# fabriceo/AVDSP

Hardware: NVIDIA B200
Metric: channel-samples/sec (higher is better)
Workload: dtype int64

## Files before the change

avdsp_b200/csrc/api.cu:

```cuda
#include "../../include/avdsp_b200.h"
#include "decoder.h"
#include "kernels.h"
#include "host_numa.h"
#include <cuda_runtime.h>
#include <algorithm>
#include <cstdio>
#include <cstdlib>
#include <cstring>
#include <memory>
#include <map>
#include <mutex>
#include <string>
#include <thread>
#include <vector>

using namespace avdsp;

static thread_local std::string g_lastError;
static int setErr(int code, const std::string& msg) { g_lastError = msg; return code; }
static int cudaErr(cudaError_t e, const char* what) {
    return setErr(AVDSP_B200_ERR_CUDA, std::string(what) + ": " + cudaGetErrorString(e));
}
#define NO_MULTI(h, what) do { if (!(h)->shards.empty()) return setErr(AVDSP_B200_ERR_UNSUPPORTED, what " takes a single-device instance (device buffers belong to one GPU)"); } while (0)
#define CU(call) do { cudaError_t e_ = (call); if (e_ != cudaSuccess) return cudaErr(e_, #call); } while (0)
// ... 77 lines not shown
__global__ void k_widen_pcm(const unsigned char* __restrict__ src, int fmt, int* __restrict__ dst, size_t n) {
    const size_t i = (size_t)blockIdx.x * blockDim.x + threadIdx.x;
    if (i >= n) return;
    int v;
    if (fmt == AVDSP_B200_PCM_S16) v = (int)((const short*)src)[i] << 16;
    else { const unsigned char* p = src + 3 * i; v = (int)(((unsigned)p[0] << 8) | ((unsigned)p[1] << 16) | ((unsigned)p[2] << 24)); }
    dst[i] = v;
}

#include "instance.h"

static int quiesce(avdsp_b200* h);
static int resetShards(avdsp_b200* h, int fs, const int32_t* seeds, int defaultDither);

static void planGeometries(avdsp_b200* h, std::vector<ChainLane>* lanes2) {
    const Lowered& L = h->L;
    h->chain2Usable = false;
    lanes2->assign(1024, ChainLane{});
    if (L.chainOk && chain2Supports(L.chain)) h->chain2Usable = planChain2Geometry(L.chain, h->nStreams, h->numSMs, &h->geom2, lanes2->data());
    h->chain3Usable = h->chain2Usable && planChain3Geometry(L.chain, h->nStreams, h->numSMs, &h->geom3);
    h->mixUsable = false;
    if (L.chainOk) { std::string why; h->mixUsable = buildMixPlan(L.chain, &h->mix, &why); }
    h->firUsable = L.firOk;
    h->dagUsable = L.dagOk && L.dag && planDagGeometry(*L.dag, h->nStreams, h->numSMs, &h->geomDag);
    char line[512];
    h->trace = L.trace;
    if (h->firUsable) {
        snprintf(line, sizeof line, "time-parallel FIR kernel: usable (%d paths, longest impulse %d taps)\n", L.fir.nPaths, L.fir.maxLen);
        h->trace += line;
    } else if (!L.firs.empty()) h->trace += "FIR kernel not used: " + L.firWhyNot + "\n";
    if (h->mixUsable) h->trace += "time-parallel mix kernel: usable (no biquad in any path)\n";
    if (h->chain2Usable) {
        snprintf(line, sizeof line, "chain kernel v2 geometry: %d streams/CTA, %d sections/lane, tile %d frames, gmax %d, %d section threads + %d helper threads, %d sources, %zu B smem\n",
                 h->geom2.streamsPerCta, h->geom2.secPerLane, h->geom2.tileFrames, h->geom2.gmax, h->geom2.secThreads, h->geom2.helpThreads, L.chain.h.nSrc, h->geom2.smemBytes);
        h->trace += line;
    }
    if (h->chain3Usable) {
        snprintf(line, sizeof line, "chain kernel v3 geometry: %d streams/CTA (lane = one cascade part of one stream), %d cascade warps of <= %d sections + 1 dither warp + %d store warps, largest lag %d frames, row ring %d steps, %zu B smem; parts (chain:first+n@base):",
                 h->geom3.streamsPerCta, h->geom3.nCascade, h->geom3.maxSec, h->geom3.nStore, h->geom3.gmax, h->geom3.postRing, h->geom3.smemBytes);
        h->trace += line;
        for (int w = 0; w < h->geom3.nCascade; w++) {
            snprintf(line, sizeof line, " %d:%d+%d@%d", h->geom3.warpChain[w], h->geom3.warpFirstSec[w], h->geom3.warpNsec[w], h->geom3.warpBase[w]);
            h->trace += line;
        }
        h->trace += "; sub-partitions (sections of the cascade warps on hardware warps q, q+4, ..; d = dither warp, s = store warp):";
        for (int q = 0; q < 4; q++) {
            h->trace += q ? " |" : " ";
            for (int id = q; id < h->geom3.threads / 32; id += 4) {
                const int role = h->geom3.warpRole[id];
                if (role >= 0) snprintf(line, sizeof line, " %d", h->geom3.warpNsec[role]);
                else snprintf(line, sizeof line, " %s", role == -1 ? "d" : "s");
                h->trace += line;
            }
        }
        h->trace += "\n";
    }
    if (h->dagUsable) {
        snprintf(line, sizeof line, "DAG kernel geometry: %d nodes (depth %d, longest cascade %d sections), %d streams/CTA, %d threads, tiles of %d frames, input rows of %d frames, %d words/stream, %zu B smem%s\n",
                 L.dag->nNodes, L.dag->maxDepth, L.dag->maxSec, h->geomDag.streamsPerCta, h->geomDag.threads, h->geomDag.tileFrames, h->geomDag.rawMask + 1, h->geomDag.perStreamWords,
                 h->geomDag.smemBytes, (h->chain2Usable || h->mixUsable || h->firUsable) ? " (another fused kernel takes this program first)" : "");
        h->trace += line;
    } else if (!L.dagOk && !h->chain2Usable && !h->mixUsable && !h->firUsable) h->trace += "DAG kernel not used: " + L.dagWhyNot + "\n";
    if (!h->chain2Usable && !h->mixUsable) {
        const bool coefRange = L.chainOk && L.chain.h.aluClass == ALU_F32 && !chainFloatCoefsInRange(L.chain);
        snprintf(line, sizeof line, "chain kernels not used: %s\n",
                 coefRange ? "a biquad coefficient lies outside [2^-60, 2^7): the float class could not bound its products (exactness guard), the interpreter runs this program"
                           : L.chainOk ? "geometry does not fit" : L.chainWhyNot.c_str());
        h->trace += line;
    }
}

static int uploadPlanData(avdsp_b200* h) {
    cudaSetDevice(h->device);
    const Lowered& L = h->L;
    if (h->dBig) { cudaFree(h->dBig); h->dBig = nullptr; }
    h->bigWords = L.bigPool.size();
    if (h->bigWords) {
        CU(cudaMalloc(&h->dBig, h->bigWords * 4));
        CU(cudaMemcpy(h->dBig, L.bigPool.data(), h->bigWords * 4, cudaMemcpyHostToDevice));
    }
    std::vector<ChainLane> lanes2;
    planGeometries(h, &lanes2);
    if (h->chain2Usable) {
        if (!h->dLanes2) CU(cudaMalloc(&h->dLanes2, 1024 * sizeof(ChainLane)));
        CU(cudaMemcpy(h->dLanes2, lanes2.data(), 1024 * sizeof(ChainLane), cudaMemcpyHostToDevice));
    }
    if (h->dFirTaps) { cudaFree(h->dFirTaps); h->dFirTaps = nullptr; }
    if (h->firUsable) {
        std::vector<unsigned char> blobs;
        firTcBuildTaps(L.fir, L.fir.aluClass == ALU_INT64 ? FIRTC_I8 : FIRTC_TF32, L.bigPool.data(), &blobs);
        CU(cudaMalloc(&h->dFirTaps, blobs.size()));
        CU(cudaMemcpy(h->dFirTaps, blobs.data(), blobs.size(), cudaMemcpyHostToDevice));
    }
    return 0;
}

static int initState(avdsp_b200* h) {
    cudaSetDevice(h->device);
    const PlanHeader& P = h->L.gen.h;
    const size_t words = (size_t)h->nStreams * P.stateWords;
    CU(cudaMemsetAsync(h->dState, 0, words * 4, h->stream));
    std::vector<int32_t> memInit(2 * std::max(P.nMem, 1), 0);
    for (int k = 0; k < P.nMem; k++) {
        memInit[2 * k] = h->L.words[h->L.memWord[k]];
        memInit[2 * k + 1] = h->L.words[h->L.memWord[k] + 1];
    }
// ... 999 lines not shown
```

avdsp_b200/csrc/kernel_chain3.cu:

```cuda
#include "avdsp_dev.cuh"
#include "kernels.h"
#include <algorithm>
#include <cstdlib>

namespace avdsp {
namespace {

constexpr int F3 = 32;
constexpr int TP3 = 4 * F3 + 1;
constexpr int kBarFull3 = 1;
constexpr int kBarDone3 = 3;
#ifndef AVDSP_UNR3
#define AVDSP_UNR3 6
#endif
constexpr unsigned kSatBias3  = (1u << (kMantBQ - 1)) - 2u;
constexpr unsigned kSatLimit3 = (1u << kMantBQ) - 3u;

__device__ __forceinline__ void barSync3(int id, int n)   { __syncwarp(); asm volatile("bar.sync %0, %1;" :: "r"(id), "r"(n) : "memory"); }
__device__ __forceinline__ void barArrive3(int id, int n) { __syncwarp(); asm volatile("bar.arrive %0, %1;" :: "r"(id), "r"(n) : "memory"); }
__device__ __forceinline__ unsigned smemAddr3(const void* p) { return (unsigned)__cvta_generic_to_shared(p); }
__device__ __forceinline__ int lds3(unsigned a) { int v; asm volatile("ld.shared.b32 %0, [%1];" : "=r"(v) : "r"(a) : "memory"); return v; }
__device__ __forceinline__ void sts3(unsigned a, int v) { asm volatile("st.shared.b32 [%0], %1;" :: "r"(a), "r"(v) : "memory"); }
__device__ __forceinline__ void mbarInit3(unsigned bar, int count) {
    asm volatile("mbarrier.init.shared::cta.b64 [%0], %1;" :: "r"(bar), "r"(count) : "memory");
}
__device__ __forceinline__ void mbarExpectTx3(unsigned bar, unsigned bytes) {
    asm volatile("mbarrier.arrive.expect_tx.shared::cta.b64 _, [%0], %1;" :: "r"(bar), "r"(bytes) : "memory");
}
__device__ __forceinline__ void tmaLoad3(unsigned dst, const void* src, unsigned bytes, unsigned bar) {
    asm volatile("cp.async.bulk.shared::cluster.global.mbarrier::complete_tx::bytes [%0], [%1], %2, [%3];"
                 :: "r"(dst), "l"(src), "r"(bytes), "r"(bar) : "memory");
}
__device__ __forceinline__ void mbarWait3(unsigned bar, unsigned parity) {
    asm volatile("{\n"
                 ".reg .pred P1;\n"
                 "WAIT3_%=:\n"
                 "mbarrier.try_wait.parity.shared::cta.b64 P1, [%0], %1;\n"
                 "@P1 bra DONE3_%=;\n"
                 "bra WAIT3_%=;\n"
                 "DONE3_%=:\n"
                 "}" :: "r"(bar), "r"(parity) : "memory");
}

template <int NSEC>
struct Casc {
    long long acc[NSEC];
    int y1[NSEC], y2[NSEC], y3[NSEC];
    int X1, X2;
    int rx1[NSEC], rx2[NSEC];
    int b0[NSEC], b1[NSEC], b2[NSEC], a1[NSEC], a2[NSEC];
};

template <int NSEC>
__device__ __forceinline__ long long cascStep(Casc<NSEC>& L, int xin, unsigned& w0, unsigned& w1) {
    long long acc[NSEC];
#pragma unroll
    for (int k = 0; k < NSEC; k++) acc[k] = mac32(L.acc[k], k ? L.y2[k - 1] : L.X1, L.b1[k]);
#pragma unroll
    for (int k = 0; k < NSEC; k++) acc[k] = mac32(acc[k], k ? L.y3[k - 1] : L.X2, L.b2[k]);
#pragma unroll
    for (int k = 0; k < NSEC; k++) acc[k] = mac32(acc[k], L.y1[k], L.a1[k]);
#pragma unroll
    for (int k = 0; k < NSEC; k++) acc[k] = mac32(acc[k], L.y2[k], L.a2[k]);
#pragma unroll
    for (int k = 0; k < NSEC; k++) acc[k] = mac32(acc[k], k ? L.y1[k - 1] : xin, L.b0[k]);
#pragma unroll
    for (int k = 0; k < NSEC; k++) {
        if (k & 1) w1 = max(w1, (unsigned)hi32(acc[k]) + kSatBias3);
        else       w0 = max(w0, (unsigned)hi32(acc[k]) + kSatBias3);
        L.acc[k] = acc[k];
        L.y3[k] = L.y2[k]; L.y2[k] = L.y1[k]; L.y1[k] = q59ToS31(acc[k]);
    }
    L.X2 = L.X1; L.X1 = xin;
    return acc[NSEC - 1];
}
template <int NSEC>
__device__ __forceinline__ long long cascStepExact(Casc<NSEC>& L, int xin, int t, int T) {
    int in[NSEC], x1[NSEC], x2[NSEC];
#pragma unroll
    for (int k = 0; k < NSEC; k++) {
        const int f = t - k;
        in[k] = k ? L.y1[k - 1] : xin;
        x1[k] = k ? (f == 0 ? L.rx1[k] : L.y2[k - 1]) : L.X1;
        x2[k] = k ? (f == 0 ? L.rx2[k] : (f == 1 ? L.rx1[k] : L.y3[k - 1])) : L.X2;
    }
    long long last = 0;
#pragma unroll
    for (int k = 0; k < NSEC; k++) {
        if ((unsigned)(t - k) < (unsigned)T) {
            long long acc = L.acc[k];
            acc = mac32(acc, x1[k], L.b1[k]);
            acc = mac32(acc, x2[k], L.b2[k]);
            acc = mac32(acc, L.y1[k], L.a1[k]);
            acc = mac32(acc, L.y2[k], L.a2[k]);
            acc = mac32(acc, in[k], L.b0[k]);
            acc = biquadSat(acc);
            L.acc[k] = acc;
            L.y3[k] = L.y2[k]; L.y2[k] = L.y1[k]; L.y1[k] = q59ToS31(acc);
            if (k == NSEC - 1) last = acc;
        }
    }
    if ((unsigned)t < (unsigned)T) { L.X2 = L.X1; L.X1 = xin; }
    return last;
}

__device__ __forceinline__ int finishTpdf3(long long acc, int tv, bool up, int sh) {
    const long long t = tv;
    acc += up ? (long long)((unsigned long long)t << sh) : (t >> sh);
    return sat64_031_s32(acc);
}

template <int NSEC, int MODE, bool CKREG>
__device__ __forceinline__ void cascadeWarp(const ChainPlan& P, const Chain2Args& A, const Chain3Geom& G, unsigned char* smem,
                                            int w, int lane) {
    constexpr int LAG = NSEC - 1;
    const int NS = G.streamsPerCta, W = P.h.stateWords, T = A.nFrames;
    const int s0 = blockIdx.x * NS, nsHere = min(NS, A.nStreams - s0);
    const int c = G.warpChain[w];
    const ChainDesc& d = P.chains[c];
    const int sec0 = G.warpFirstSec[w];
    const int base = G.warpBase[w];
    const int LAGA = base + LAG;
    const int srcWarp = G.warpSrc[w];
    const bool fin = G.warpFinal[w] != 0;
    const bool live = lane < nsHere;
    const int sl = min(lane, nsHere - 1);
    const int RM = G.postRing - 1;
    const unsigned RM4 = (unsigned)RM << 2, TM4 = (unsigned)(4 * F3 - 1) << 2;
    const unsigned sb = smemAddr3(smem);
    const unsigned postRow = sb + (unsigned)G.warpRowOff[w] + (unsigned)(sl * G.warpPitch[w]) * 4u;
    const unsigned srcRow = sb + (unsigned)G.warpRowOff[max(srcWarp, 0)] + (unsigned)(sl * G.warpPitch[max(srcWarp, 0)]) * 4u;
    volatile int* tileDone = reinterpret_cast<volatile int*>(smem + G.doneOff);
    const unsigned tpdfRow = sb + G.tpdfOff + (unsigned)(sl * TP3) * 4u;
    const unsigned rawRow = sb + G.rawOff + (unsigned)(sl * G.rawPitchBytes) + (unsigned)d.srcCh * 4u;
    const unsigned fb = (unsigned)P.h.nIn * 4u;
    const unsigned mbar = sb + G.mbarOff;
    const int gain = srcWarp >= 0 ? (1 << kMant) : (d.srcKind == SRC_LOAD_GAIN ? d.srcArg : 1);
    const bool tpdfUp = P.h.tpdfShift >= 0;
    const int tpdfSh = (tpdfUp ? P.h.tpdfShift : -P.h.tpdfShift) & 63;
    const bool wantTpdf = fin && (d.satKind & 1) != 0;
    int* st = A.state + (size_t)(s0 + sl) * W;

    Casc<NSEC> L;
    L.X1 = L.X2 = 0;
#pragma unroll
    for (int k = 0; k < NSEC; k++) {
        const int* cf = P.pool + d.coefOff + 5 * (sec0 + k);
        L.b0[k] = cf[0]; L.b1[k] = cf[1]; L.b2[k] = cf[2]; L.a1[k] = cf[3]; L.a2[k] = cf[4];
        L.y3[k] = 0;
        {
            const int* q = st + P.pool[d.secStateOff + sec0 + k];
            L.acc[k] = (long long)(((unsigned long long)(unsigned)q[1] << 32) | (unsigned)q[0]);
            L.rx1[k] = q[2]; L.rx2[k] = q[3]; L.y1[k] = q[4]; L.y2[k] = q[5];
            if (k == 0) { L.X1 = q[2]; L.X2 = q[3]; }
        }
    }
    const int n = fin ? d.delayN : 0;
    int idx0 = 0, staleIdx = -1;
    if (live && n > 0) {
        const int* ring = st + d.delayOff + 1;
        idx0 = st[d.delayOff];
        const bool stale = idx0 >= n || idx0 < 0;
        for (int k = 0; k < n; k++) {
            const int v = !stale ? ring[(idx0 + k) % n] : (k == 0 ? ring[idx0] : ring[k - 1]);
            sts3(postRow + ((unsigned)((k - n + LAGA) & RM) << 2), v);
        }
        if (stale) { sts3(postRow + ((unsigned)(LAGA & RM) << 2), ring[n - 1]); staleIdx = idx0; idx0 = n - 1; }
    }
    const bool anyStale = __any_sync(0xffffffffu, staleIdx >= 0);
    int* ck = reinterpret_cast<int*>(smem + G.ckOff) + (w * 32 + lane);
    const int CKP = G.nCascade * 32;
    const int nTiles = (T + G.gmax + F3 - 1) / F3;

    for (int i = 0; i < nTiles; i++) {
        barSync3(kBarFull3 + (i & 1), G.threads);
        const int t0 = i * F3;
        unsigned ra, rstep;
        if (srcWarp < 0) {
            if (G.tma && t0 + F3 <= T) mbarWait3(mbar + 8u * (unsigned)(i & 1), (unsigned)((i >> 1) & 1));
            ra = rawRow + (unsigned)(i & 1) * (unsigned)G.rawStageBytes; rstep = fb;
        } else {
            if (i > 0) { while (tileDone[srcWarp] < i) { } __threadfence_block(); __syncwarp(); }
            ra = srcRow + (unsigned)(((i + 2) % 3) * F3) * 4u; rstep = 4u;
        }
        const int tl0 = t0 - base;
        bool exact = !(tl0 >= LAG + 2 && tl0 + F3 <= T && !(anyStale && tl0 <= LAG));
        if (!exact) {
            long long cAcc[CKREG ? NSEC : 1]; int cY1[CKREG ? NSEC : 1], cY2[CKREG ? NSEC : 1], cY3[CKREG ? NSEC : 1], cX1 = 0, cX2 = 0;
            if (CKREG) {
#pragma unroll
                for (int k = 0; k < NSEC; k++) { cAcc[CKREG ? k : 0] = L.acc[k]; cY1[CKREG ? k : 0] = L.y1[k]; cY2[CKREG ? k : 0] = L.y2[k]; cY3[CKREG ? k : 0] = L.y3[k]; }
                cX1 = L.X1; cX2 = L.X2;
            } else {
#pragma unroll
                for (int k = 0; k < NSEC; k++) {
                    ck[(5 * k + 0) * CKP] = lo32(L.acc[k]); ck[(5 * k + 1) * CKP] = hi32(L.acc[k]);
                    ck[(5 * k + 2) * CKP] = L.y1[k]; ck[(5 * k + 3) * CKP] = L.y2[k]; ck[(5 * k + 4) * CKP] = L.y3[k];
                }
                ck[(5 * NSEC) * CKP] = L.X1; ck[(5 * NSEC + 1) * CKP] = L.X2;
            }
            unsigned w0 = 0, w1 = 0;
            unsigned rj = ra;
            unsigned pj = postRow + (fin ? ((unsigned)(t0 & RM) << 2) : (unsigned)((i % 3) * F3) * 4u);
            unsigned tj = (unsigned)((t0 - LAGA) << 2);
            auto step = [&](int jj) {
                const int smp = lds3(rj); rj += rstep;
                const int x = (MODE & 1) ? smp : q59ToS31(mul32(smp, gain));
                const long long acc = cascStep<NSEC>(L, x, w0, w1);
                int v;
                if (MODE & 2) v = finishTpdf3(acc, lds3(tpdfRow + ((tj + 4u * jj) & TM4)), tpdfUp, tpdfSh);
                else v = q59ToS31(acc);
                if (live) sts3(pj + 4u * jj, v);
            };
            constexpr int kMain = (F3 / AVDSP_UNR3) * AVDSP_UNR3;
#pragma unroll 1
            for (int j0 = 0; j0 < kMain; j0 += AVDSP_UNR3) {
#pragma unroll
                for (int jj = 0; jj < AVDSP_UNR3; jj++) step(jj);
                pj += 4u * AVDSP_UNR3; tj += 4u * AVDSP_UNR3;
            }
#pragma unroll
            for (int jj = 0; jj < F3 - kMain; jj++) step(jj);
            if (__any_sync(0xffffffffu, max(w0, w1) > kSatLimit3)) {
                if (CKREG) {
#pragma unroll
                    for (int k = 0; k < NSEC; k++) { L.acc[k] = cAcc[CKREG ? k : 0]; L.y1[k] = cY1[CKREG ? k : 0]; L.y2[k] = cY2[CKREG ? k : 0]; L.y3[k] = cY3[CKREG ? k : 0]; }
                    L.X1 = cX1; L.X2 = cX2;
                } else {
#pragma unroll
                    for (int k = 0; k < NSEC; k++) {
                        L.acc[k] = (long long)(((unsigned long long)(unsigned)ck[(5 * k + 1) * CKP] << 32) | (unsigned)ck[(5 * k + 0) * CKP]);
                        L.y1[k] = ck[(5 * k + 2) * CKP]; L.y2[k] = ck[(5 * k + 3) * CKP]; L.y3[k] = ck[(5 * k + 4) * CKP];
                    }
                    L.X1 = ck[(5 * NSEC) * CKP]; L.X2 = ck[(5 * NSEC + 1) * CKP];
                }
                exact = true;
            }
        }
        if (exact) {
#pragma unroll 1
            for (int j = 0; j < F3; j++) {
                const int t = t0 + j, tl = t - base;
                if (tl >= T + LAG) break;
                if (tl < 0) continue;
                const int smp = tl < T ? lds3(ra + (unsigned)j * rstep) : 0;
                const int x = q59ToS31(mul32(smp, gain));
                const long long acc = cascStepExact<NSEC>(L, x, tl, T);
                const int f = tl - LAG;
                if (f >= 0) {
                    int v;
                    if (wantTpdf) v = finishTpdf3(acc, lds3(tpdfRow + ((unsigned)(f << 2) & TM4)), tpdfUp, tpdfSh);
                    else v = q59ToS31(acc);
                    if (live) {
                        if (f == 0 && staleIdx >= 0) st[d.delayOff + 1 + staleIdx] = v;
                        else sts3(postRow + (fin ? ((unsigned)(t << 2) & RM4) : (unsigned)((i % 3) * F3 + j) * 4u), v);
                    }
                }
            }
        }
        if (!fin) {
            __syncwarp();
            if (lane == 0) { __threadfence_block(); tileDone[w] = i + 1; }
        }
        barArrive3(kBarDone3 + (i & 1), G.threads);
    }

    if (live) {
#pragma unroll
        for (int k = 0; k < NSEC; k++) {
            int* q = st + P.pool[d.secStateOff + sec0 + k];
            q[0] = lo32(L.acc[k]); q[1] = hi32(L.acc[k]);
            if (k == 0) { q[2] = L.X1; q[3] = L.X2; }
            else if (T >= 2) { q[2] = L.y1[k - 1]; q[3] = L.y2[k - 1]; }
            else if (T == 1) { q[2] = L.y1[k - 1]; q[3] = L.rx1[k]; }
            q[4] = L.y1[k]; q[5] = L.y2[k];
        }
// ... 253 lines not shown
                if (f >= 0) {
                    const int v = emit(acc, f);
                    if (live) {
                        if (f == 0 && staleIdx >= 0) st[d.delayOff + 1 + staleIdx] = v;
                        else sts3(postRow + (fin ? ((unsigned)(t << 2) & RM4) : (unsigned)((i % 3) * F3 + j) * 4u), v);
                    }
                }
            }
        }
        if (!fin) {
            __syncwarp();
            if (lane == 0) { __threadfence_block(); tileDone[w] = i + 1; }
        }
        barArrive3(kBarDone3 + (i & 1), G.threads);
    }
    if (live) {
#pragma unroll
        for (int k = 0; k < NSEC; k++) {
            int* q = st + P.pool[d.secStateOff + sec0 + k];
            q[0] = __float_as_int(L.acc[k]);
            if (k == 0) { q[2] = __float_as_int(L.X1); q[3] = __float_as_int(L.X2); }
            else if (T >= 2) { q[2] = __float_as_int(L.y1[k - 1]); q[3] = __float_as_int(L.y2[k - 1]); }
            else if (T == 1) { q[2] = __float_as_int(L.y1[k - 1]); q[3] = __float_as_int(L.rx1[k]); }
            q[4] = __float_as_int(L.y1[k]); q[5] = __float_as_int(L.y2[k]);
        }
        if (fltGuardFired(mn) && A.redo) A.redo[s0 + sl] = 1;
        if (n > 0 && T > 0) {
            int* ring = st + d.delayOff + 1;
            for (int k = 0; k < n; k++) {
                const long long j = (long long)T - n + k;
                ring[(int)(((long long)idx0 + j + n) % n)] = __float_as_int(satF(__int_as_float(lds3(postRow + ((unsigned)(((int)j + LAGA) & RM) << 2)))));
            }
            st[d.delayOff] = (int)(((long long)idx0 + T) % n);
        }
    }
}
template <int NSEC>
__device__ __forceinline__ void cascadeWarpFin(const ChainPlan& P, const Chain2Args& A, const Chain3Geom& G, unsigned char* smem, int w, int lane) {
    const int finm = !G.warpFinal[w] ? 0 : (P.chains[G.warpChain[w]].satKind & 1) ? 2 : 1;
    const int src = G.warpSrc[w] >= 0 ? 1 : (P.h.sampleInt ? 0 : 2);
    switch (finm * 3 + src) {
    case 0:  cascadeWarpF<NSEC, 0, 0>(P, A, G, smem, w, lane); break;
    case 1:  cascadeWarpF<NSEC, 0, 1>(P, A, G, smem, w, lane); break;
    case 2:  cascadeWarpF<NSEC, 0, 2>(P, A, G, smem, w, lane); break;
    case 3:  cascadeWarpF<NSEC, 1, 0>(P, A, G, smem, w, lane); break;
    case 4:  cascadeWarpF<NSEC, 1, 1>(P, A, G, smem, w, lane); break;
    case 5:  cascadeWarpF<NSEC, 1, 2>(P, A, G, smem, w, lane); break;
    case 6:  cascadeWarpF<NSEC, 2, 0>(P, A, G, smem, w, lane); break;
    case 7:  cascadeWarpF<NSEC, 2, 1>(P, A, G, smem, w, lane); break;
    default: cascadeWarpF<NSEC, 2, 2>(P, A, G, smem, w, lane); break;
    }
}

template <int NSEC, bool CKREG>
__device__ __forceinline__ void cascadeWarpMode(const ChainPlan& P, const Chain2Args& A, const Chain3Geom& G, unsigned char* smem,
                                                int w, int lane, int mode) {
    switch (mode) {
    case 0:  cascadeWarp<NSEC, 0, CKREG>(P, A, G, smem, w, lane); break;
    case 1:  cascadeWarp<NSEC, 1, CKREG>(P, A, G, smem, w, lane); break;
    case 2:  cascadeWarp<NSEC, 2, CKREG>(P, A, G, smem, w, lane); break;
    default: cascadeWarp<NSEC, 3, CKREG>(P, A, G, smem, w, lane); break;
    }
}

template <bool FLT, bool FSMP> __device__ __forceinline__ int post3(int v) {
    if (FLT) return FSMP ? __float_as_int(satF(__int_as_float(v))) : f2s31SatFast(v);
    return v;
}

template <int NOUT, bool FLT, bool FSMP>
__device__ __forceinline__ void storeTile3(int* __restrict__ out, unsigned rowA, unsigned p4, unsigned RM4, int mask, bool clean,
                                           int f0, int fs, int T) {
    constexpr int FPP = 32 / NOUT, NPASS = F3 / FPP;
    if (clean) {
#pragma unroll
        for (int p = 0; p < NPASS; p++) out[p * 32] = post3<FLT, FSMP>(lds3(rowA + ((p4 + (unsigned)(p * FPP * 4)) & RM4))) & mask;
    } else {
#pragma unroll 1
        for (int p = 0; p < NPASS; p++) {
            const int f = f0 + p * FPP + fs;
            if (f >= 0 && f < T) out[p * 32] = post3<FLT, FSMP>(lds3(rowA + ((p4 + (unsigned)(p * FPP * 4)) & RM4))) & mask;
        }
    }
}

template <int NOUT, bool FLT, bool FSMP>
__device__ __forceinline__ void storeStreams3(int* __restrict__ out, size_t outStep, unsigned rowA, unsigned rowStep, int cnt, unsigned p4,
                                              unsigned RM4, int mask, bool clean, int f0, int fs, int T) {
#pragma unroll 1
    for (int s = 0; s < cnt; s++, out += outStep, rowA += rowStep) storeTile3<NOUT, FLT, FSMP>(out, rowA, p4, RM4, mask, clean, f0, fs, T);
}

}

template <int MAXSEC, bool FLT = false>
__global__ void __launch_bounds__(MAXSEC > 4 ? kChain3MaxThreads : kChain3MaxThreadsParts, 1)
k_chain3(const __grid_constant__ ChainPlan P, const Chain2Args A, const __grid_constant__ Chain3Geom G) {
    extern __shared__ __align__(128) unsigned char smem_raw[];
    const int lane = threadIdx.x & 31;
    const int role = G.warpRole[threadIdx.x >> 5];
    if constexpr (FLT) {
        if (role >= 0) {
            switch (G.warpNsec[role]) {
            case 1: cascadeWarpFin<1>(P, A, G, smem_raw, role, lane); break;
            case 2: cascadeWarpFin<2>(P, A, G, smem_raw, role, lane); break;
            case 3: cascadeWarpFin<3>(P, A, G, smem_raw, role, lane); break;
            default: cascadeWarpFin<4>(P, A, G, smem_raw, role, lane); break;
            }
            return;
        }
    } else if (role >= 0) {
        const int warp = role;
        const ChainDesc& d = P.chains[G.warpChain[warp]];
        const bool unity = G.warpSrc[warp] >= 0 || (d.srcKind == SRC_LOAD_GAIN && d.srcArg == (1 << kMant));
        const int mode = (unity ? 1 : 0) | ((G.warpFinal[warp] && (d.satKind & 1)) ? 2 : 0);
        switch (G.warpNsec[warp]) {
        case 1: cascadeWarpMode<1, (MAXSEC <= 4)>(P, A, G, smem_raw, warp, lane, mode); break;
        case 2: cascadeWarpMode<2, (MAXSEC <= 4)>(P, A, G, smem_raw, warp, lane, mode); break;
        case 3: cascadeWarpMode<3, (MAXSEC <= 4)>(P, A, G, smem_raw, warp, lane, mode); break;
        case 4: cascadeWarpMode<4, (MAXSEC <= 4)>(P, A, G, smem_raw, warp, lane, mode); break;
        default:
            if constexpr (MAXSEC > 4) {
                switch (G.warpNsec[warp]) {
                case 5: cascadeWarpMode<5, (MAXSEC <= 4)>(P, A, G, smem_raw, warp, lane, mode); break;
                case 6: cascadeWarpMode<6, (MAXSEC <= 4)>(P, A, G, smem_raw, warp, lane, mode); break;
                case 7: cascadeWarpMode<7, (MAXSEC <= 4)>(P, A, G, smem_raw, warp, lane, mode); break;
                default: cascadeWarpMode<8, (MAXSEC <= 4)>(P, A, G, smem_raw, warp, lane, mode); break;
                }
            }
            break;
        }
        return;
    }
    const int NS = G.streamsPerCta, W = P.h.stateWords, T = A.nFrames;
    const int s0 = blockIdx.x * NS, nsHere = min(NS, A.nStreams - s0);
    const int gmax = G.gmax;
    const int nTiles = (T + gmax + F3 - 1) / F3;
    const int hw = -role - 1;
    const unsigned sb = smemAddr3(smem_raw);
    const unsigned RM4 = (unsigned)(G.postRing - 1) << 2;

    if (hw == 0) {
        const bool own = lane < nsHere;
        const bool hasCalc = P.h.hasTpdfCalc != 0;
        const int nIn = P.h.nIn;
        Prng g = {0, 0, 0, 0}; int tpdfValue = 0, tpdfRandom = 0, dith = 0; bool drew = false;
        int* auxp = nullptr;
        if (own) {
            auxp = A.state + (size_t)(s0 + lane) * W + P.h.auxOff;
            g.s0 = auxp[AUX_S0]; g.s1 = auxp[AUX_S1]; g.s2 = auxp[AUX_S2]; g.s3 = auxp[AUX_S3];
            tpdfValue = auxp[AUX_TPDF_VALUE]; tpdfRandom = auxp[AUX_TPDF_RANDOM]; dith = auxp[AUX_DITHER];
        }
        const unsigned mbar = sb + G.mbarOff;
        const unsigned rowBytes = (unsigned)(F3 * nIn * 4);
        if (G.tma && lane == 0) { mbarInit3(mbar, 1); mbarInit3(mbar + 8, 1); asm volatile("fence.mbarrier_init.release.cluster;" ::: "memory"); }
        if (lane < kChain3MaxWarps) reinterpret_cast<volatile int*>(smem_raw + G.doneOff)[lane] = 0;
        __syncwarp();
        auto issueTile = [&](int it) {
            if (!G.tma || (it + 1) * F3 > T) return;
            asm volatile("fence.proxy.async.shared::cta;" ::: "memory");
            const unsigned bar = mbar + 8u * (unsigned)(it & 1);
            if (lane == 0) mbarExpectTx3(bar, (unsigned)nsHere * rowBytes);
            __syncwarp();
            if (own) {
                const int* src = A.in + (size_t)(s0 + lane) * A.inStreamStride + (size_t)(it * F3) * A.inFrameStride;
                tmaLoad3(sb + G.rawOff + (unsigned)(it & 1) * (unsigned)G.rawStageBytes + (unsigned)(lane * G.rawPitchBytes), src, rowBytes, bar);
            }
        };
        auto copyTile = [&](int it) {
            const int f0 = it * F3;
            if (f0 >= T || (G.tma && f0 + F3 <= T)) return;
            const int nf = min(F3, T - f0);
            const unsigned dst0 = sb + G.rawOff + (unsigned)(it & 1) * (unsigned)G.rawStageBytes;
            for (int s = 0; s < nsHere; s++) {
                const int* src = A.in + (size_t)(s0 + s) * A.inStreamStride + (size_t)f0 * A.inFrameStride;
                for (int e = lane; e < nf * nIn; e += 32) {
                    const int fr = e / nIn, ch = e - fr * nIn;
                    sts3(dst0 + (unsigned)(s * G.rawPitchBytes) + 4u * (unsigned)e, src[(size_t)fr * A.inFrameStride + (size_t)ch * A.inChStride]);
                }
            }
        };
        auto ditherTile = [&](int it) {
            const int f0 = it * F3;
// ... 60 lines not shown
                case 4:  storeStreams3<4, FLT, true>(out, outStep, rowA, rowStep, cnt, p4, RM4, bMask, clean, f0, bFs, T); break;
                case 8:  storeStreams3<8, FLT, true>(out, outStep, rowA, rowStep, cnt, p4, RM4, bMask, clean, f0, bFs, T); break;
                case 16: storeStreams3<16, FLT, true>(out, outStep, rowA, rowStep, cnt, p4, RM4, bMask, clean, f0, bFs, T); break;
                default: storeStreams3<32, FLT, true>(out, outStep, rowA, rowStep, cnt, p4, RM4, bMask, clean, f0, bFs, T); break;
                }
            } else {
                switch (nOut) {
                case 1:  storeStreams3<1, FLT, false>(out, outStep, rowA, rowStep, cnt, p4, RM4, bMask, clean, f0, bFs, T); break;
                case 2:  storeStreams3<2, FLT, false>(out, outStep, rowA, rowStep, cnt, p4, RM4, bMask, clean, f0, bFs, T); break;
                case 4:  storeStreams3<4, FLT, false>(out, outStep, rowA, rowStep, cnt, p4, RM4, bMask, clean, f0, bFs, T); break;
                case 8:  storeStreams3<8, FLT, false>(out, outStep, rowA, rowStep, cnt, p4, RM4, bMask, clean, f0, bFs, T); break;
                case 16: storeStreams3<16, FLT, false>(out, outStep, rowA, rowStep, cnt, p4, RM4, bMask, clean, f0, bFs, T); break;
                default: storeStreams3<32, FLT, false>(out, outStep, rowA, rowStep, cnt, p4, RM4, bMask, clean, f0, bFs, T); break;
                }
            }
        } else {
            const int f = f0 + lane;
            if (f >= 0 && f < T)
                for (int sl = sw; sl < nsHere; sl += nSW)
                    for (int ch = 0; ch < nOut; ch++) {
                        const int oc = P.h.chainOfOut[ch];
                        int v = 0;
                        if (oc >= 0) {
                            const int off = G.chainLag[oc] - P.chains[oc].delayN;
                            { const int wv_ = lds3(sb + (unsigned)G.warpRowOff[G.chainRow[oc]] + (unsigned)(sl * G.postPitch) * 4u + ((unsigned)((f + off) << 2) & RM4)); v = (fsmp ? post3<FLT, true>(wv_) : post3<FLT, false>(wv_)) & storeMask; }
                        }
                        A.out[(size_t)(s0 + sl) * A.outStreamStride + (size_t)f * A.outFrameStride + (size_t)ch * A.outChStride] = v;
                    }
        }
    }
}

static int envInt3(const char* name, int dflt) { const char* v = getenv(name); return (v && *v) ? atoi(v) : dflt; }

bool chain3Supports(const ChainPlan& plan) {
    const ChainHeader& h = plan.h;
    if (h.aluClass != ALU_INT64 && h.aluClass != ALU_F32) return false;
    if (h.aluClass == ALU_F32 && !chainFloatCoefsInRange(plan)) return false;
    if (h.nChains <= 0 || h.nChains > kChain3MaxChains || h.nIn <= 0) return false;
    if (h.nOut <= 0 || h.nOut > 32 || (h.nOut & (h.nOut - 1)) != 0) return false;
    if (h.nRaw || h.nDelayFirst || h.nMemCopy) return false;
    for (int c = 0; c < h.nChains; c++) {
        const ChainDesc& d = plan.chains[c];
        if (d.nsec < 1 || d.nsec > 16) return false;
        if (d.srcKind != SRC_LOAD && d.srcKind != SRC_LOAD_GAIN) return false;
        if (d.srcCh < 0 || d.srcCh >= h.nIn) return false;
        if (d.hasGain || d.delayFirst) return false;
        if (d.satKind != SAT_PLAIN && d.satKind != SAT_TPDF) return false;
        if (d.delayN < 0) return false;
    }
    return true;
}

bool planChain3Geometry(const ChainPlan& plan, int nStreams, int numSMs, Chain3Geom* geom) {
    if (!chain3Supports(plan)) return false;
    const int C = plan.h.nChains;
    int NS = envInt3("AVDSP_B200_NS3", 0);
    if (NS <= 0) NS = (nStreams + numSMs - 1) / numSMs;
    NS = std::max(1, std::min(NS, 32));
    int maxDelay = 0;
    for (int c = 0; c < C; c++) maxDelay = std::max(maxDelay, plan.chains[c].delayN);
    for (int partMax : {envInt3("AVDSP_B200_PART3", 4), 8}) {
        if (partMax < 1 || partMax > 8) continue;
        if (plan.h.aluClass == ALU_F32 && partMax > 4) continue;
        struct Part { int chain, first, nsec, base, src, fin; };
        Part parts[kChain3MaxWarps];
        int nParts = 0, gmax = 0, maxSec = 0;
        bool fits = true;
        Chain3Geom g{};
        for (int c = 0; c < C && fits; c++) {
            const int nsec = plan.chains[c].nsec, np = (nsec + partMax - 1) / partMax;
            if (np > ((plan.chains[c].satKind & 1) ? 2 : 4)) { fits = false; break; }
            int first = 0, base = 0, prev = -1;
            for (int p = 0; p < np; p++) {
                if (nParts >= kChain3MaxWarps) { fits = false; break; }
                const int n = nsec / np + (p < nsec % np ? 1 : 0);
                parts[nParts] = {c, first, n, base, prev, p == np - 1};
                prev = nParts++;
                first += n;
                maxSec = std::max(maxSec, n);
                gmax = std::max(gmax, base + n - 1);
                if (p == np - 1) g.chainLag[c] = base + n - 1;
                base += n - 1 + F3;
            }
        }
        if (!fits) continue;
        const int maxThreads = maxSec > 4 ? kChain3MaxThreads : kChain3MaxThreadsParts;
        g.streamsPerCta = NS;
        g.floatFast = 1;
        for (int c = 0; c < C; c++)
            if (plan.chains[c].srcKind == SRC_LOAD_GAIN) {
                const int ex = (int)(((uint32_t)plan.chains[c].srcArg >> 23) & 255u);
                if (ex != 0 && (ex < 127 - 30 || ex > 127 + 30)) g.floatFast = 0;
            }
        if (envInt3("AVDSP_B200_FLOAT_EXACT_HELPERS", 0)) g.floatFast = 0;
        g.nCascade = nParts;
        g.gmax = gmax;
        g.maxSec = maxSec;
        g.nStore = std::max(1, std::min(envInt3("AVDSP_B200_SW3", plan.h.aluClass == ALU_F32 ? 4 : 3), maxThreads / 32 - nParts - 1));
        g.threads = (nParts + 1 + g.nStore) * 32;
        if (g.threads > maxThreads) continue;
        int R = 2 * F3;
        while (R < 2 * F3 + gmax + maxDelay) R <<= 1;
        g.postRing = R; g.postPitch = R + 1;
        g.rawPitchBytes = F3 * plan.h.nIn * 4 + 16;
        g.rawStageBytes = NS * g.rawPitchBytes;
// ... 1 lines not shown
            const int total = nParts + 1 + g.nStore;
            int slots[4];
            for (int q = 0; q < 4; q++) slots[q] = (total - q + 3) / 4;
            int itemCost[32], itemBin[32], order[32];
            for (int k = 0; k < total; k++) {
                order[k] = k;
                if (k >= nParts) { itemCost[k] = 8; continue; }
                const ChainDesc& d = plan.chains[parts[k].chain];
                itemCost[k] = 5 * parts[k].nsec + 2;
                if (parts[k].fin && (d.satKind & 1)) itemCost[k] += 6;
                if (parts[k].src < 0 && !(d.srcKind == SRC_LOAD_GAIN && d.srcArg == (1 << kMant))) itemCost[k] += 2;
            }
            std::stable_sort(order, order + total, [&](int a, int b) { return itemCost[a] > itemCost[b]; });
            int binCost[4] = {0, 0, 0, 0}, used[4] = {0, 0, 0, 0};
            for (int k = 0; k < total; k++) {
                int best = -1;
                for (int q = 0; q < 4; q++) if (used[q] < slots[q] && (best < 0 || binCost[q] < binCost[best])) best = q;
                itemBin[order[k]] = best; used[best]++; binCost[best] += itemCost[order[k]];
            }
            for (int iter = 0; iter < 64; iter++) {
                int ba = -1, bb = -1; long long bestGain = 0;
                for (int a = 0; a < total; a++)
                    for (int b = a + 1; b < total; b++) {
                        const int qa = itemBin[a], qb = itemBin[b];
                        if (qa == qb || itemCost[a] == itemCost[b]) continue;
                        const int dlt = itemCost[a] - itemCost[b];
                        const long long before = (long long)binCost[qa] * binCost[qa] + (long long)binCost[qb] * binCost[qb];
                        const long long after = (long long)(binCost[qa] - dlt) * (binCost[qa] - dlt) + (long long)(binCost[qb] + dlt) * (binCost[qb] + dlt);
                        if (before - after > bestGain) { bestGain = before - after; ba = a; bb = b; }
                    }
                if (ba < 0) break;
                const int qa = itemBin[ba], qb = itemBin[bb], dlt = itemCost[ba] - itemCost[bb];
                binCost[qa] -= dlt; binCost[qb] += dlt;
                itemBin[ba] = qb; itemBin[bb] = qa;
            }
            if (const char* ov = getenv("AVDSP_B200_BINS3")) {
                int k = 0;
                for (const char* q = ov; *q && k < total; q++) if (*q >= '0' && *q <= '3') itemBin[k++] = *q - '0';
                int cnt[4] = {0, 0, 0, 0};
                for (int kk = 0; kk < total; kk++) cnt[itemBin[kk]]++;
                for (int q = 0; q < 4; q++) if (cnt[q] != slots[q]) return false;
            }
            int next[4] = {0, 0, 0, 0};
            for (int k = 0; k < 32; k++) g.warpRole[k] = -1;
            int slotOf[kChain3MaxWarps];
            for (int k = 0; k < total; k++) {
                const int id = itemBin[k] + 4 * next[itemBin[k]]++;
                if (k < nParts) { slotOf[k] = k; g.warpRole[id] = k; } else g.warpRole[id] = -1 - (k - nParts);
            }
            for (int k = 0; k < nParts; k++) {
                const int w = slotOf[k];
                g.warpChain[w] = parts[k].chain; g.warpFirstSec[w] = parts[k].first; g.warpNsec[w] = parts[k].nsec;
                g.warpBase[w] = parts[k].base; g.warpSrc[w] = parts[k].src >= 0 ? slotOf[parts[k].src] : -1; g.warpFinal[w] = parts[k].fin;
                if (parts[k].fin) g.chainRow[parts[k].chain] = w;
            }
        }
        size_t bytes = 0;
        g.postOff = 0;
        for (int w = 0; w < nParts; w++) {
            g.warpPitch[w] = g.warpFinal[w] ? g.postPitch : 3 * F3 + 1;
            g.warpRowOff[w] = (int)bytes; bytes += (size_t)NS * g.warpPitch[w] * 4;
        }
        g.tpdfOff = (int)bytes; bytes += (size_t)NS * TP3 * 4;
        g.ckOff = (int)bytes;   if (maxSec > 4) bytes += (size_t)(5 * maxSec + 2) * nParts * 32 * 4;
        g.doneOff = (int)bytes; bytes += (size_t)kChain3MaxWarps * 4;
        bytes = (bytes + 15) & ~(size_t)15;
        g.mbarOff = (int)bytes; bytes += 16;
        bytes = (bytes + 127) & ~(size_t)127;
        g.rawOff = (int)bytes;  bytes += (size_t)2 * g.rawStageBytes;
        g.smemBytes = bytes + 16;
        if (g.smemBytes > 226 * 1024) continue;
        *geom = g;
        return true;
    }
    return false;
}

static bool chain3TmaOk(const ChainPlan& plan, const Chain2Args& a) {
    const int nIn = plan.h.nIn;
    return a.inChStride == 1 && a.inFrameStride == nIn && ((size_t)a.in & 15) == 0 && (a.inStreamStride & 3) == 0 && ((F3 * nIn * 4) & 15) == 0;
}

cudaError_t launchChain3(const ChainPlan& plan, const Chain3Geom& geom, const Chain2Args& args, cudaStream_t stream) {
    Chain3Geom g = geom;
    g.tma = chain3TmaOk(plan, args) ? 1 : 0;
    const int blocks = (args.nStreams + g.streamsPerCta - 1) / g.streamsPerCta;
    cudaError_t e;
    if (plan.h.aluClass == ALU_F32) {
        e = cudaFuncSetAttribute(k_chain3<4, true>, cudaFuncAttributeMaxDynamicSharedMemorySize, (int)g.smemBytes);
        if (e != cudaSuccess) return e;
        k_chain3<4, true><<<blocks, g.threads, g.smemBytes, stream>>>(plan, args, g);
    } else if (g.maxSec > 4) {
        e = cudaFuncSetAttribute(k_chain3<8>, cudaFuncAttributeMaxDynamicSharedMemorySize, (int)g.smemBytes);
        if (e != cudaSuccess) return e;
        k_chain3<8><<<blocks, g.threads, g.smemBytes, stream>>>(plan, args, g);
    } else {
        e = cudaFuncSetAttribute(k_chain3<4>, cudaFuncAttributeMaxDynamicSharedMemorySize, (int)g.smemBytes);
        if (e != cudaSuccess) return e;
        k_chain3<4><<<blocks, g.threads, g.smemBytes, stream>>>(plan, args, g);
    }
    return cudaGetLastError();
}

}
```

avdsp_b200/csrc/kernels.h:

```cpp
#pragma once
#include <cuda_runtime.h>
#include <string>
#include <vector>
#include "plan.h"

namespace avdsp {

constexpr int kGenericThreads = 128;

struct GenericArgs {
    const int* in;  int* out;
    int* state;
    const int* bigPool;
    int nStreams, nFrames;
    long long inStreamStride, outStreamStride;
    int inFrameStride, inChStride, outFrameStride, outChStride;
    int coreSel;
    int period;
    int stageState;
    const int* redo;
    const int* snapshot;
    unsigned coreInMask[kMaxCores], coreOutMask[kMaxCores];
};
cudaError_t launchGeneric(const GenericPlan& plan, const GenericArgs& args, cudaStream_t stream);
// ... 39 lines not shown
    int exact;
};
cudaError_t launchRedoPrepare(const int* state, int* snapshot, size_t words, int* flags, int nStreams, int* count, cudaStream_t stream);
cudaError_t launchRedoCompact(const int* flags, int nStreams, int* list, int* count, int* state, const int* snapshot, int stateWords, cudaStream_t stream);
bool chainFloatCoefsInRange(const ChainPlan& plan);
bool chain2Supports(const ChainPlan& plan);
bool planChain2Geometry(const ChainPlan& plan, int nStreams, int numSMs, Chain2Geom* geom, ChainLane* lanesOut );
cudaError_t launchChain2(const ChainPlan& plan, const Chain2Geom& geom, const Chain2Args& args, cudaStream_t stream);

constexpr int kDagMaxThreads = 384;
struct DagGeom {
    int streamsPerCta;
    int threads, nStore;
    int tileFrames;
    int perStreamWords;
    int rawOff, rawMask;
    int tpdfOff, tpdfMask;
    int nRawOut;
    int rawOutCh[kIoSlots], rawOutSrc[kIoSlots];
    int accMask[kMaxDagNodes];
    int staleOff;
    int tabOff;
    int accLoOff[kMaxDagNodes], accHiOff[kMaxDagNodes];
    int postOff[kMaxDagNodes], postMask[kMaxDagNodes];
    int aDlyOff[kMaxDagNodes], aDlyMask[kMaxDagNodes];
    int bDlyOff[kMaxDagNodes], bDlyMask[kMaxDagNodes];
    size_t smemBytes;
};
struct Chain2Args;
bool planDagGeometry(const DagPlan& plan, int nStreams, int numSMs, DagGeom* geom);
cudaError_t launchDag(const DagPlan& plan, const DagGeom& geom, const Chain2Args& args, cudaStream_t stream);

constexpr int kChain3MaxChains = 10;
constexpr int kChain3MaxWarps = 16;
constexpr int kChain3MaxThreads = 384;
constexpr int kChain3MaxThreadsParts = 512;
struct Chain3Geom {
    int streamsPerCta;
    int nCascade;
    int nStore;
    int gmax;
    int maxSec;
    int threads;
    int postRing;
    int postPitch;
    int rawPitchBytes, rawStageBytes;
    int postOff, tpdfOff, ckOff, doneOff, mbarOff, rawOff;
    int tma;
    int floatFast;
    int warpChain[kChain3MaxWarps], warpFirstSec[kChain3MaxWarps], warpNsec[kChain3MaxWarps];
    int warpBase[kChain3MaxWarps];
    int warpSrc[kChain3MaxWarps];
    int warpFinal[kChain3MaxWarps];
    int warpRowOff[kChain3MaxWarps];
    int warpPitch[kChain3MaxWarps];
    int warpRole[32];
    int chainRow[kChain3MaxChains];
    int chainLag[kChain3MaxChains];
    size_t smemBytes;
};
bool chain3Supports(const ChainPlan& plan);
bool planChain3Geometry(const ChainPlan& plan, int nStreams, int numSMs, Chain3Geom* geom);
cudaError_t launchChain3(const ChainPlan& plan, const Chain3Geom& geom, const Chain2Args& args, cudaStream_t stream);

struct MixPlan {
    int nIn, nOut, nChains, nInPad;
    int stateWords, auxOff;
    int hasCalc, tpdfDither, tpdfDataOff, tpdfShift, anyTpdf;
    int storeMask, maxDelay;
    int cDelay[kFastTab], cDelayOff[kFastTab], cMuxOff[kFastTab], cOut[kFastTab];
    int oChain[kFastTab], oDelay[kFastTab], oDelayOff[kFastTab], oFlags[kFastTab], oGain[kFastTab], oSatGain[kFastTab],
        oKind[kFastTab], oSrcCh[kFastTab], oMatRow[kFastTab], oDelayBytes[kFastTab], oDelayPcmBytes[kFastTab];
    int uniform, uFlags;
    int mat[kFastTab * kFastTab];
};
struct MixArgs {
    const int* in;  int* out;
    int* state;
    int* tpdfBuf;
    int nStreams, nFrames;
    long long inStreamStride, outStreamStride;
    int inFrameStride, inChStride, outFrameStride, outChStride;
    int vecIn, vecOut;
    int tileFrames, winFrames;
};
bool buildMixPlan(const ChainPlan& plan, MixPlan* out, std::string* why);
void mixJumpMatrix(long long steps, unsigned* out );
constexpr int kMixJumpLevels = 8;
void mixPrngSegments(const MixPlan& M, const MixArgs& A, int numSMs, int* J, int* L);
cudaError_t launchMix(const MixPlan& M, MixArgs A, const unsigned* dJump, int J, int L, int numSMs, cudaStream_t stream, int* launches);

struct FirArgs {
    const int* in;  int* out;
    int* state;
    const int* bigPool;
    int nStreams, nFrames;
    long long inStreamStride, outStreamStride;
    int inFrameStride, inChStride, outFrameStride, outChStride;
};
cudaError_t launchFir(const FirPlan& plan, const FirArgs& args, int numSMs, cudaStream_t stream, int* launches);
cudaError_t launchFirState(const FirPlan& plan, const FirArgs& args, cudaStream_t stream);

enum FirTcKind : int { FIRTC_I8 = 0 , FIRTC_TF32 = 1  };
int firTcHistory(const FirPlan& plan);
void firTcBuildTaps(const FirPlan& plan, int kind, const int32_t* bigPool, std::vector<unsigned char>* out);
size_t firTcWorkspaceBytes(const FirPlan& plan, int kind, int nStreams, int nFrames);
// ... 5 lines not shown
```

Measured before the change: 182,600.

## Use error-feedback form for unit-DC-gain biquad sections in chain3 cascade

```diff
diff --git a/avdsp_b200/csrc/api.cu b/avdsp_b200/csrc/api.cu
--- a/avdsp_b200/csrc/api.cu
+++ b/avdsp_b200/csrc/api.cu
@@ -153,6 +153,13 @@
                 else snprintf(line, sizeof line, " %s", role == -1 ? "d" : "s");
                 h->trace += line;
             }
+        }
+        h->trace += "\n";
+        h->trace += "chain kernel v3 section forms (chain:first+n):";
+        for (int w = 0; w < h->geom3.nCascade; w++) {
+            snprintf(line, sizeof line, " %d:%d+%d=", h->geom3.warpChain[w], h->geom3.warpFirstSec[w], h->geom3.warpNsec[w]);
+            h->trace += line;
+            for (int k = 0; k < h->geom3.warpNsec[w]; k++) h->trace += (h->geom3.warpUnit[w] >> k) & 1 ? "u" : "g";
         }
         h->trace += "\n";
     }
diff --git a/avdsp_b200/csrc/kernel_chain3.cu b/avdsp_b200/csrc/kernel_chain3.cu
--- a/avdsp_b200/csrc/kernel_chain3.cu
+++ b/avdsp_b200/csrc/kernel_chain3.cu
@@ -49,30 +49,82 @@
     int X1, X2;
     int rx1[NSEC], rx2[NSEC];
     int b0[NSEC], b1[NSEC], b2[NSEC], a1[NSEC], a2[NSEC];
+    int e1[NSEC], e2[NSEC];
 };
 
-template <int NSEC>
-__device__ __forceinline__ long long cascStep(Casc<NSEC>& L, int xin, unsigned& w0, unsigned& w1) {
+struct UnitRec { unsigned wa = 0u; int ov = 0; int ym = 0x7FFFFFFF; };
+constexpr unsigned kUnitBias3  = 1u << (kMantBQ - 1);
+constexpr unsigned kUnitLimit3 = (1u << kMantBQ) - 1u;
+constexpr int kUnitYMin3 = (int)0x80000000 + 32;
+__device__ __forceinline__ bool unitFired(const UnitRec& r) { return r.wa > kUnitLimit3 || r.ov < 0 || r.ym < kUnitYMin3; }
+
+template <int NSEC, int UM, bool WANTACC>
+__device__ __forceinline__ long long cascStep(Casc<NSEC>& L, int xin, unsigned& w0, unsigned& w1, UnitRec& ur) {
     long long acc[NSEC];
 #pragma unroll
-    for (int k = 0; k < NSEC; k++) acc[k] = mac32(L.acc[k], k ? L.y2[k - 1] : L.X1, L.b1[k]);
-#pragma unroll
-    for (int k = 0; k < NSEC; k++) acc[k] = mac32(acc[k], k ? L.y3[k - 1] : L.X2, L.b2[k]);
-#pragma unroll
-    for (int k = 0; k < NSEC; k++) acc[k] = mac32(acc[k], L.y1[k], L.a1[k]);
-#pragma unroll
-    for (int k = 0; k < NSEC; k++) acc[k] = mac32(acc[k], L.y2[k], L.a2[k]);
-#pragma unroll
-    for (int k = 0; k < NSEC; k++) acc[k] = mac32(acc[k], k ? L.y1[k - 1] : xin, L.b0[k]);
+    for (int k = 0; k < NSEC; k++) acc[k] = (UM >> k) & 1 ? mac32(L.acc[k], L.e1[k], L.a1[k]) : mac32(L.acc[k], k ? L.y2[k - 1] : L.X1, L.b1[k]);
+#pragma unroll
+    for (int k = 0; k < NSEC; k++) acc[k] = (UM >> k) & 1 ? mac32(acc[k], L.e2[k], L.a2[k]) : mac32(acc[k], k ? L.y3[k - 1] : L.X2, L.b2[k]);
+#pragma unroll
+    for (int k = 0; k < NSEC; k++) if (!((UM >> k) & 1)) acc[k] = mac32(acc[k], L.y1[k], L.a1[k]);
+#pragma unroll
+    for (int k = 0; k < NSEC; k++) if (!((UM >> k) & 1)) acc[k] = mac32(acc[k], L.y2[k], L.a2[k]);
+#pragma unroll
+    for (int k = 0; k < NSEC; k++) if (!((UM >> k) & 1)) acc[k] = mac32(acc[k], k ? L.y1[k - 1] : xin, L.b0[k]);
+    int in[NSEC];
+#pragma unroll
+    for (int k = 0; k < NSEC; k++) in[k] = k ? L.y1[k - 1] : xin;
+    long long last = 0;
 #pragma unroll
     for (int k = 0; k < NSEC; k++) {
-        if (k & 1) w1 = max(w1, (unsigned)hi32(acc[k]) + kSatBias3);
-        else       w0 = max(w0, (unsigned)hi32(acc[k]) + kSatBias3);
+        int y;
+        if ((UM >> k) & 1) {
+            const int x = in[k];
+            const int e = q59ToS31(acc[k]);
+            y = e + x;
+            ur.wa = max(ur.wa, (unsigned)hi32(acc[k]) + kUnitBias3);
+            ur.ov |= (e ^ y) & (x ^ y);
+            ur.ym = min(ur.ym, y);
+            L.e2[k] = L.e1[k]; L.e1[k] = e;
+            if (WANTACC && k == NSEC - 1) last = mac32(acc[k], x, 1 << kMantBQ);
+        } else {
+            if (k & 1) w1 = max(w1, (unsigned)hi32(acc[k]) + kSatBias3);
+            else       w0 = max(w0, (unsigned)hi32(acc[k]) + kSatBias3);
+            y = q59ToS31(acc[k]);
+            if (WANTACC && k == NSEC - 1) last = acc[k];
+        }
         L.acc[k] = acc[k];
-        L.y3[k] = L.y2[k]; L.y2[k] = L.y1[k]; L.y1[k] = q59ToS31(acc[k]);
+        L.y3[k] = L.y2[k]; L.y2[k] = L.y1[k]; L.y1[k] = y;
     }
     L.X2 = L.X1; L.X1 = xin;
-    return acc[NSEC - 1];
+    return last;
+}
+template <int NSEC, int UM>
+__device__ __forceinline__ bool unitFits(const Casc<NSEC>& L) {
+    bool ok = true;
+#pragma unroll
+    for (int k = 0; k < NSEC; k++)
+        if ((UM >> k) & 1) {
+            const long long d1 = (long long)L.y1[k] - (k ? L.y2[k - 1] : L.X1), d2 = (long long)L.y2[k] - (k ? L.y3[k - 1] : L.X2);
+            ok = ok && d1 == (long long)(int)d1 && d2 == (long long)(int)d2;
+        }
+    return ok;
+}
+template <int NSEC, int UM>
+__device__ __forceinline__ void unitEnter(Casc<NSEC>& L) {
+#pragma unroll
+    for (int k = 0; k < NSEC; k++)
+        if ((UM >> k) & 1) {
+            const int x1 = k ? L.y2[k - 1] : L.X1, x2 = k ? L.y3[k - 1] : L.X2;
+            L.acc[k] -= (long long)x1 << kMantBQ;
+            L.e1[k] = L.y1[k] - x1; L.e2[k] = L.y2[k] - x2;
+        }
+}
+template <int NSEC, int UM>
+__device__ __forceinline__ void unitLeave(Casc<NSEC>& L) {
+#pragma unroll
+    for (int k = 0; k < NSEC; k++)
+        if ((UM >> k) & 1) L.acc[k] += (long long)(k ? L.y2[k - 1] : L.X1) << kMantBQ;
 }
 template <int NSEC>
 __device__ __forceinline__ long long cascStepExact(Casc<NSEC>& L, int xin, int t, int T) {
@@ -110,7 +162,7 @@
     return sat64_031_s32(acc);
 }
 
-template <int NSEC, int MODE, bool CKREG>
+template <int NSEC, int MODE, bool CKREG, int UM>
 __device__ __forceinline__ void cascadeWarp(const ChainPlan& P, const Chain2Args& A, const Chain3Geom& G, unsigned char* smem,
                                             int w, int lane) {
     constexpr int LAG = NSEC - 1;
@@ -185,6 +237,7 @@
         }
         const int tl0 = t0 - base;
         bool exact = !(tl0 >= LAG + 2 && tl0 + F3 <= T && !(anyStale && tl0 <= LAG));
+        if (UM && !exact && __any_sync(0xffffffffu, !unitFits<NSEC, UM>(L))) exact = true;
         if (!exact) {
             long long cAcc[CKREG ? NSEC : 1]; int cY1[CKREG ? NSEC : 1], cY2[CKREG ? NSEC : 1], cY3[CKREG ? NSEC : 1], cX1 = 0, cX2 = 0;
             if (CKREG) {
@@ -200,16 +253,18 @@
                 ck[(5 * NSEC) * CKP] = L.X1; ck[(5 * NSEC + 1) * CKP] = L.X2;
             }
             unsigned w0 = 0, w1 = 0;
+            UnitRec ur;
+            if (UM) unitEnter<NSEC, UM>(L);
             unsigned rj = ra;
             unsigned pj = postRow + (fin ? ((unsigned)(t0 & RM) << 2) : (unsigned)((i % 3) * F3) * 4u);
             unsigned tj = (unsigned)((t0 - LAGA) << 2);
             auto step = [&](int jj) {
                 const int smp = lds3(rj); rj += rstep;
                 const int x = (MODE & 1) ? smp : q59ToS31(mul32(smp, gain));
-                const long long acc = cascStep<NSEC>(L, x, w0, w1);
+                const long long acc = cascStep<NSEC, UM, (MODE & 2) != 0>(L, x, w0, w1, ur);
                 int v;
                 if (MODE & 2) v = finishTpdf3(acc, lds3(tpdfRow + ((tj + 4u * jj) & TM4)), tpdfUp, tpdfSh);
-                else v = q59ToS31(acc);
+                else v = L.y1[NSEC - 1];
                 if (live) sts3(pj + 4u * jj, v);
             };
             constexpr int kMain = (F3 / AVDSP_UNR3) * AVDSP_UNR3;
@@ -221,7 +276,8 @@
             }
 #pragma unroll
             for (int jj = 0; jj < F3 - kMain; jj++) step(jj);
-            if (__any_sync(0xffffffffu, max(w0, w1) > kSatLimit3)) {
+            if (UM) unitLeave<NSEC, UM>(L);
+            if (__any_sync(0xffffffffu, max(w0, w1) > kSatLimit3 || (UM && unitFired(ur)))) {
                 if (CKREG) {
 #pragma unroll
                     for (int k = 0; k < NSEC; k++) { L.acc[k] = cAcc[CKREG ? k : 0]; L.y1[k] = cY1[CKREG ? k : 0]; L.y2[k] = cY2[CKREG ? k : 0]; L.y3[k] = cY3[CKREG ? k : 0]; }
@@ -581,15 +637,22 @@
     }
 }
 
-template <int NSEC, bool CKREG>
+template <int NSEC, bool CKREG, int UM = 0>
 __device__ __forceinline__ void cascadeWarpMode(const ChainPlan& P, const Chain2Args& A, const Chain3Geom& G, unsigned char* smem,
                                                 int w, int lane, int mode) {
     switch (mode) {
-    case 0:  cascadeWarp<NSEC, 0, CKREG>(P, A, G, smem, w, lane); break;
-    case 1:  cascadeWarp<NSEC, 1, CKREG>(P, A, G, smem, w, lane); break;
-    case 2:  cascadeWarp<NSEC, 2, CKREG>(P, A, G, smem, w, lane); break;
-    default: cascadeWarp<NSEC, 3, CKREG>(P, A, G, smem, w, lane); break;
-    }
+    case 0:  cascadeWarp<NSEC, 0, CKREG, UM>(P, A, G, smem, w, lane); break;
+    case 1:  cascadeWarp<NSEC, 1, CKREG, UM>(P, A, G, smem, w, lane); break;
+    case 2:  cascadeWarp<NSEC, 2, CKREG, UM>(P, A, G, smem, w, lane); break;
+    default: cascadeWarp<NSEC, 3, CKREG, UM>(P, A, G, smem, w, lane); break;
+    }
+}
+template <int NSEC, int UM = (1 << NSEC) - 1>
+__device__ __forceinline__ void cascadeWarpUnit(const ChainPlan& P, const Chain2Args& A, const Chain3Geom& G, unsigned char* smem,
+                                                int w, int lane, int mode, int um) {
+    if constexpr (UM == 0) cascadeWarpMode<NSEC, true, 0>(P, A, G, smem, w, lane, mode);
+    else if (um == UM) cascadeWarpMode<NSEC, true, UM>(P, A, G, smem, w, lane, mode);
+    else cascadeWarpUnit<NSEC, UM - 1>(P, A, G, smem, w, lane, mode, um);
 }
 
 template <bool FLT, bool FSMP> __device__ __forceinline__ int post3(int v) {
@@ -643,21 +706,25 @@
         const ChainDesc& d = P.chains[G.warpChain[warp]];
         const bool unity = G.warpSrc[warp] >= 0 || (d.srcKind == SRC_LOAD_GAIN && d.srcArg == (1 << kMant));
         const int mode = (unity ? 1 : 0) | ((G.warpFinal[warp] && (d.satKind & 1)) ? 2 : 0);
-        switch (G.warpNsec[warp]) {
-        case 1: cascadeWarpMode<1, (MAXSEC <= 4)>(P, A, G, smem_raw, warp, lane, mode); break;
-        case 2: cascadeWarpMode<2, (MAXSEC <= 4)>(P, A, G, smem_raw, warp, lane, mode); break;
-        case 3: cascadeWarpMode<3, (MAXSEC <= 4)>(P, A, G, smem_raw, warp, lane, mode); break;
-        case 4: cascadeWarpMode<4, (MAXSEC <= 4)>(P, A, G, smem_raw, warp, lane, mode); break;
-        default:
-            if constexpr (MAXSEC > 4) {
-                switch (G.warpNsec[warp]) {
-                case 5: cascadeWarpMode<5, (MAXSEC <= 4)>(P, A, G, smem_raw, warp, lane, mode); break;
-                case 6: cascadeWarpMode<6, (MAXSEC <= 4)>(P, A, G, smem_raw, warp, lane, mode); break;
-                case 7: cascadeWarpMode<7, (MAXSEC <= 4)>(P, A, G, smem_raw, warp, lane, mode); break;
-                default: cascadeWarpMode<8, (MAXSEC <= 4)>(P, A, G, smem_raw, warp, lane, mode); break;
-                }
-            }
-            break;
+        if constexpr (MAXSEC <= 4) {
+            const int um = G.warpUnit[warp];
+            switch (G.warpNsec[warp]) {
+            case 1: cascadeWarpUnit<1>(P, A, G, smem_raw, warp, lane, mode, um); break;
+            case 2: cascadeWarpUnit<2>(P, A, G, smem_raw, warp, lane, mode, um); break;
+            case 3: cascadeWarpUnit<3>(P, A, G, smem_raw, warp, lane, mode, um); break;
+            default: cascadeWarpUnit<4>(P, A, G, smem_raw, warp, lane, mode, um); break;
+            }
+        } else {
+            switch (G.warpNsec[warp]) {
+            case 1: cascadeWarpMode<1, false>(P, A, G, smem_raw, warp, lane, mode); break;
+            case 2: cascadeWarpMode<2, false>(P, A, G, smem_raw, warp, lane, mode); break;
+            case 3: cascadeWarpMode<3, false>(P, A, G, smem_raw, warp, lane, mode); break;
+            case 4: cascadeWarpMode<4, false>(P, A, G, smem_raw, warp, lane, mode); break;
+            case 5: cascadeWarpMode<5, false>(P, A, G, smem_raw, warp, lane, mode); break;
+            case 6: cascadeWarpMode<6, false>(P, A, G, smem_raw, warp, lane, mode); break;
+            case 7: cascadeWarpMode<7, false>(P, A, G, smem_raw, warp, lane, mode); break;
+            default: cascadeWarpMode<8, false>(P, A, G, smem_raw, warp, lane, mode); break;
+            }
         }
         return;
     }
@@ -824,6 +891,10 @@
     return true;
 }
 
+static bool unitGainSection(const int32_t* cf) {
+    return cf[0] == (1 << kMantBQ) && (long long)cf[1] == -((long long)cf[3] + (1ll << kMantBQ)) && (long long)cf[2] == -(long long)cf[4];
+}
+
 bool planChain3Geometry(const ChainPlan& plan, int nStreams, int numSMs, Chain3Geom* geom) {
     if (!chain3Supports(plan)) return false;
     const int C = plan.h.nChains;
@@ -931,6 +1002,12 @@
                 const int w = slotOf[k];
                 g.warpChain[w] = parts[k].chain; g.warpFirstSec[w] = parts[k].first; g.warpNsec[w] = parts[k].nsec;
                 g.warpBase[w] = parts[k].base; g.warpSrc[w] = parts[k].src >= 0 ? slotOf[parts[k].src] : -1; g.warpFinal[w] = parts[k].fin;
+                g.warpUnit[w] = 0;
+                if (plan.h.aluClass == ALU_INT64 && maxSec <= 4 && envInt3("AVDSP_B200_UNIT3", 1)) {
+                    const int* cf = plan.pool + plan.chains[parts[k].chain].coefOff + 5 * parts[k].first;
+                    for (int j = 0; j < parts[k].nsec; j++) if (unitGainSection(cf + 5 * j)) g.warpUnit[w] |= 1 << j;
+                    if (envInt3("AVDSP_B200_UNIT3", 1) == 2 && g.warpUnit[w] != (1 << parts[k].nsec) - 1) g.warpUnit[w] = 0;
+                }
                 if (parts[k].fin) g.chainRow[parts[k].chain] = w;
             }
         }
diff --git a/avdsp_b200/csrc/kernels.h b/avdsp_b200/csrc/kernels.h
--- a/avdsp_b200/csrc/kernels.h
+++ b/avdsp_b200/csrc/kernels.h
@@ -115,6 +115,7 @@
     int warpBase[kChain3MaxWarps];
     int warpSrc[kChain3MaxWarps];
     int warpFinal[kChain3MaxWarps];
+    int warpUnit[kChain3MaxWarps];
     int warpRowOff[kChain3MaxWarps];
     int warpPitch[kChain3MaxWarps];
     int warpRole[32];
```

Result: slower. 136,400, median of 6 (-25.3%).
